# L-Scofano/SEEME

Measured on AMD Instinct MI355X. Metric: sampled seqs/sec (T=196, 50 DDIM steps), higher is better.
Workload: dtype f32 accumulate (fp16 denoiser weights, fp16 VAE MFMA operands); 1 GPU; config_mld_egobody interactee-only: VAE encode -> 50-step DDIM -> VAE decode, B=32/GPU, T=196, nfeats=132, random-init recipe weights; batch_per_gpu=32, seq_len=196, ddim_steps=50, parallelism=dp1 (independent shards, no collective on the data path)

## Files before the change

seeme_amd/csrc/den_cluster.inc.hip:

```cpp

#define DCL_MAGIC_EPOCH 0x7fffffffu
#define DCL_SPIN_LIMIT (1u << 22)

typedef __attribute__((address_space(1))) unsigned long long dcl_gu64;

template <typename WT> struct ClW {
    static constexpr int KL = WT::MFMA ? 32 : 16;
    static constexpr int UL = 256 / KL;
    static constexpr int RU = WT::MFMA ? 4 : 2;
    static constexpr unsigned UNIT_BYTES = 8u * UL * 1024u;
};
template <int C, bool Q = false> struct ClG {
    static constexpr int S = 256 / C;
    static constexpr int NB = 1024 / C;
    static constexpr int TA = S / 32;
    static constexpr int TB = 8 / C;
    static constexpr int U_A = 0, U_AS = TA, U_B = 2 * TA, U_C = U_B + TB;
    static constexpr int U_G = U_C + TB, U_H = U_G + 1;
    static constexpr int U_D = Q ? U_H + 2 : U_C + TB, U_E = U_D + 1, U_F = U_E + 1, NU_REAL = U_F + 2;
    static constexpr int NU = (NU_REAL + 3) / 4 * 4;
    static constexpr int SC = Q ? 8 : 4;
    static constexpr int X1_G = 2 * S + SC;
    static constexpr int G_BOOT = 0, G_X1 = 16, G_X2 = G_X1 + C * X1_G, G_X3 = G_X2 + C * 256, G_TOTAL = G_X3 + (Q ? C * 8 : 0);
    static constexpr int EPL = Q ? 3 : 2;
// ... 110 lines not shown
    }()), ...);
}
template <typename WT, int C, bool Q, int U0, int... Is>
__device__ __forceinline__ void cl_refills(ClRing<WT>& ring, int wave, unsigned voff, __amdgpu_buffer_rsrc_t rsrc, unsigned bc, unsigned bn,
                                           bool sc, bool sn, std::integer_sequence<int, Is...>) {
    (cl_issue<WT, C, Q, U0 + Is + ClW<WT>::RU>(ring, wave, voff, rsrc, bc, bn, sc, sn), ...);
    __builtin_amdgcn_sched_barrier(0);
}
constexpr int cl_clamp(int v, int lo, int hi) { return v < lo ? lo : (v > hi ? hi : v); }

#ifndef DCL_POLL_SLEEP
#define DCL_POLL_SLEEP 12
#endif
template <int... Us> using ClSeq = std::integer_sequence<int, Us...>;
template <int C, bool MF, bool Q> struct ClSched { static constexpr bool WIN = false; static constexpr int PRO = 0; typedef ClSeq<> W1A, W1B, W2A, W2B, WXA, WXB, W3, AF; };
template <> struct ClSched<8, true, false> { static constexpr bool WIN = true; static constexpr int PRO = 2; typedef ClSeq<> WXA, WXB; typedef ClSeq<2, 3> W1A; typedef ClSeq<4> W1B; typedef ClSeq<5> W2A; typedef ClSeq<6> W2B;
                                             typedef ClSeq<7> W3; typedef ClSeq<8, 9> AF; };
template <> struct ClSched<8, true, true> { static constexpr bool WIN = true; static constexpr int PRO = 2; typedef ClSeq<2, 3> W1A; typedef ClSeq<4> W1B; typedef ClSeq<5> W2A; typedef ClSeq<6> W2B;
                                            typedef ClSeq<7> WXA; typedef ClSeq<8> WXB; typedef ClSeq<9, 10> W3; typedef ClSeq<12, 13> AF; };
template <> struct ClSched<4, true, false> { static constexpr bool WIN = true; static constexpr int PRO = 4; typedef ClSeq<4, 5> W1A; typedef ClSeq<6, 7> W1B; typedef ClSeq<8, 9> W2A; typedef ClSeq<10, 11> W2B;
                                             typedef ClSeq<> WXA, WXB; typedef ClSeq<12, 13> W3; typedef ClSeq<14, 15> AF; };
template <> struct ClSched<4, true, true> { static constexpr bool WIN = true; static constexpr int PRO = 4; typedef ClSeq<4, 5> W1A; typedef ClSeq<6, 7> W1B; typedef ClSeq<8, 9> W2A; typedef ClSeq<10> W2B;
                                            typedef ClSeq<11> WXA; typedef ClSeq<12> WXB; typedef ClSeq<13, 14> W3; typedef ClSeq<16, 17, 18, 19> AF; };
template <typename WT, int C, bool Q, int... Us>
__device__ __forceinline__ void cl_issue_seq(ClRing<WT>& ring, int wave, unsigned voff, __amdgpu_buffer_rsrc_t rsrc, unsigned bc, unsigned bn,
                                             bool sc, bool sn, ClSeq<Us...>) {
    (cl_issue<WT, C, Q, Us>(ring, wave, voff, rsrc, bc, bn, sc, sn), ...);
    __builtin_amdgcn_sched_barrier(0);
}
typedef __attribute__((address_space(3))) volatile int cl_lds_flag;
__device__ __forceinline__ void cl_flag_set(int* f, unsigned v) { *(cl_lds_flag*)f = (int)v; }
__device__ __forceinline__ void cl_flag_wait(const int* f, unsigned v) {
    while (*(const cl_lds_flag*)f != (int)v) __builtin_amdgcn_s_sleep(1);
}

__device__ __forceinline__ void cl_store_granule(unsigned long long* g, unsigned epoch, float v, bool local) {
    const unsigned long long x = ((unsigned long long)epoch << 32) | __float_as_uint(v);
    if (local) *(volatile dcl_gu64*)g = x;
    else __hip_atomic_store((dcl_gu64*)g, x, __ATOMIC_RELAXED, __HIP_MEMORY_SCOPE_AGENT);
}
__device__ __forceinline__ unsigned cl_tags_ok(const u32x4& a, unsigned epoch) { return (unsigned)(a.y == epoch) & (unsigned)(a.w == epoch); }

template <int C> struct ClRes {
    static constexpr int S = ClG<C>::S, NB = ClG<C>::NB;
    static constexpr int SKIP_B = 0, IN_B = S;
    static constexpr int L1B = 4 * S;
    static constexpr int V5 = L1B + NB;
    static constexpr int F1B = V5 + 5 * 256;
    static constexpr int V4 = F1B + FF_D;
    static constexpr int CT = V4 + 4 * 256;
    static constexpr int LAYER = CT + 512;
    static constexpr int NL1 = NB > 256 ? NB / 256 : 1;
    static constexpr int NP = 16 + NL1;
    static constexpr int ROWS = 5 * 256;
    static constexpr int FLOATS = SEEME_DEN_NL * LAYER + 2 * ROWS;
};
template <int C>
__device__ __forceinline__ void cl_load_resident(int wave, int lane, float* __restrict__ res, const float* __restrict__ vpg, const DenLayout* __restrict__ lay,
                                                 const float* __restrict__ tt_row, const SeemeSampleArgs& A, int b, int c, int ca_R) {
    typedef ClRes<C> R;
    const uint32_t base = lds_addr_of(res);
#pragma unroll 1
    for (int p = wave; p < SEEME_DEN_NL * R::NP + 5; p += DEN_THREADS / 64) {
        const float* src; int d, n = 64;
        if (p >= SEEME_DEN_NL * R::NP) {
            const int j = p - SEEME_DEN_NL * R::NP;
// ... 48 lines not shown
        else if (i <= 15) { src = tt_row + l * 512 + (i - 14) * 256; d = VP_LAYER + (i - 14) * 256; n = 64; }
        else if (i <= 17) { src = tt_row + 2560 + l * 1024 + 512 + (i - 16) * 256; d = VP_LAYER + 1024 + (i - 16) * 256; n = 64; }
        else if (i < 18 + NL1) { d = (int)(L->l1b - L->skip_b) + c * G::NB + (i - 18) * 256; src = vb + d; n = G::NB >= 256 ? 64 : G::NB / 4; }
        else {
            const int j = i - 18 - NL1;
            if (j <= 1) { src = tt_row + 2560 + l * 1024 + j * 256; d = VP_LAYER + 512 + j * 256; n = 64; }
            else if (j <= 6) {
                const int64_t f = j == 2 ? L->cnw : j == 3 ? L->cnb : j == 4 ? L->csnw : j == 5 ? L->csnb : L->cao_b;
                d = (int)(f - L->skip_b); src = vb + d; n = 64;
            }
            else if (j == 7) { d = (int)(L->caq_b - L->skip_b) + c * G::S; src = vb + d; n = G::S / 4; }
            else if (j < 8 + 4 * A.N) {
                const int t = (j - 8) >> 2, q = (j - 8) & 3;
                src = A.ctab + ((size_t)b * A.N + t) * SEEME_CROW + (q < 2 ? l * 512 + q * 256 : 2560 + l * 512 + (q - 2) * 256);
                d = VP_LAYER + STG_TT + t * 1024 + q * 256; n = 64;
            }
        }
        dst = d; n4 = n;
        r = make_float4(0.f, 0.f, 0.f, 0.f);
        if (lane < n) r = *reinterpret_cast<const float4*>(src + 4 * lane);
    }
    __device__ __forceinline__ void store(int lane, float* __restrict__ stg) const {
        if (lane < n4) *reinterpret_cast<float4*>(stg + dst + 4 * lane) = r;
    }
};
#define DCL_MAX_N 2

template <typename WT, int C, bool Q>
__global__ __launch_bounds__(DEN_THREADS) void k_den_cluster(const ClArgs ka) {
    extern __shared__ __attribute__((aligned(16))) float smem[];
    typedef ClW<WT> W; typedef ClG<C, Q> G;
    constexpr int A_DEF0 = cl_clamp(2 * G::TA - W::RU, 0, 2 * G::TA);
    constexpr int A_INL0 = cl_clamp(A_DEF0, 0, G::TA), A_INL1 = cl_clamp(A_DEF0 - G::TA, 0, G::TA), C_INL = cl_clamp(G::TB - W::RU, 0, G::TB);
    typedef ClSched<C, WT::MFMA, Q> SCH;
    constexpr bool WIN = SCH::WIN;
    const SeemeSampleArgs& A = ka.s;
    const DenLayout* __restrict__ lay = &ka.lay;
    const float* __restrict__ vp = ka.vp;
    const int tid = threadIdx.x, lane = tid & 63;
    const int wave = __builtin_amdgcn_readfirstlane(tid >> 6);
    int b, c;
    if (ka.placement == 0) { const int x = blockIdx.x & 7, j = blockIdx.x >> 3; b = x * (ka.clusters / 8) + j / C; c = j % C; }
    else { b = blockIdx.x / C; c = blockIdx.x % C; }
    if (b >= A.B) return;
    const bool epi = wave == 0;
    const int N = Q ? A.N : 1;
    typedef ClRes<C> R;
    constexpr bool RSD = !Q;
    const int stg_sz = VP_LAYER + STG_TT + N * 1024;
    const int ca_R = A.trow_per_sample ? 1 : A.steps;

    float* CONSTV = smem;
    float* KEEP = CONSTV + 768;
    float* STG = KEEP + 256;
    float* ROWS = STG + SEEME_DEN_NL * R::LAYER;
    float* XA = STG + (RSD ? R::FLOATS : 2 * stg_sz);
    float* XB = XA + 512;
    float* XH = XB + 512;
    float* SKF = XH + 2 * (G::NB > 128 ? G::NB : 128);
    float* QS = SKF + 1024;
    float* KS = QS + G::S;
    float* PART = KS + G::S;
    float* RES = PART + 256;
    int* FLG = reinterpret_cast<int*>(RES + 256);
    constexpr int XZERO = 512 + 512 + 2 * (G::NB > 128 ? G::NB : 128) + 1024;

    const __amdgpu_buffer_rsrc_t wg = __builtin_amdgcn_make_buffer_rsrc(const_cast<void*>(ka.wgc), 0, (int)ka.wgc_bytes, 0x00020000);
    unsigned long long* const xg = ka.xg + (size_t)b * G::G_TOTAL;
    const __amdgpu_buffer_rsrc_t xr_ = __builtin_amdgcn_make_buffer_rsrc(xg, 0, G::G_TOTAL * 8, 0x00020000);
    const unsigned voff = (unsigned)wave * (unsigned)(W::UL * 1024) + (unsigned)lane * 16u;
    const int col = lane & 15;
    const ClX xa = cl_xin<WT>(XA, lane), xb = cl_xin<WT>(XB, lane), xh = cl_xin<WT>(XH, lane);
    const float sa_scale = 1.f / 16.f;
    if (epi) __builtin_amdgcn_s_setprio(3);

    typedef const __attribute__((address_space(4))) int32_t* CI32;
    typedef const __attribute__((address_space(4))) float* CF32;
    const CI32 trow_c = (CI32)(uintptr_t)A.trow;
    const CF32 coef_c = (CF32)(uintptr_t)A.coef;
    int row = A.trow_per_sample ? trow_c[b] : trow_c[0];

    float4 xr = ld4(A.latents + (size_t)b * 256 + 4 * lane);
    for (int i = tid; i < 192; i += DEN_THREADS)
        st4(CONSTV + 4 * i, i < 64 ? ld4(vp + lay->pe0 + 4 * i) : (i < 128 ? ld4(vp + lay->fnw + 4 * (i - 64)) : ld4(vp + lay->fnb + 4 * (i - 128))));
    if constexpr (RSD) cl_load_resident<C>(wave, lane, STG, vp, lay, A.ttab + (size_t)row * SEEME_TROW, A, b, c, ca_R);
    else stage_dma<1, Q, 0, 0>(wave, lane, STG, vp, &lay->L[0], A.ttab + (size_t)row * SEEME_TROW, 0, A, b, N, 0, ca_R);
    for (int i = tid; i < XZERO / 4; i += DEN_THREADS) st4(XA + 4 * i, make_float4(0.f, 0.f, 0.f, 0.f));
    if (tid >= 1 && tid < 4) FLG[tid] = 0;
    bool dead = false, local = false;
    if (epi) {
        const unsigned my_xcc = __builtin_amdgcn_s_getreg(0x1814) & 15u;
        if (lane == 0) cl_store_granule(xg + G::G_BOOT + c, DCL_MAGIC_EPOCH, __uint_as_float(my_xcc), false);
        unsigned spins = 0, idv = 0;
        for (;;) {
            const unsigned long long x = __hip_atomic_load((dcl_gu64*)(xg + G::G_BOOT + (lane % C)), __ATOMIC_RELAXED, __HIP_MEMORY_SCOPE_AGENT);
            idv = (unsigned)x;
            if (__all((unsigned)(x >> 32) == DCL_MAGIC_EPOCH)) break;
            if (++spins > DCL_SPIN_LIMIT) { dead = true; if (lane == 0) atomicOr(ka.hdr, 1u); break; }
            __builtin_amdgcn_s_sleep(2);
        }
        local = !dead && __all(idv == my_xcc) && !(ka.flags & 1);
        if (lane == 0) { FLG[0] = local ? 1 : 0; if (local && c == 0) atomicAdd(ka.hdr + 1, 1u); }
    }
    wait_vmcnt0();
    __syncthreads();
    local = FLG[0] != 0;
    if (epi) {
        st4(KEEP + 4 * lane, xr);
        xr = f4_add(xr, ld4(CONSTV + 4 * lane));
        put_x<WT, 1>(XA, 0, 0, lane, xr);
        st4(RES + 4 * lane, xr);
    }
    ClRing<WT> ring;
    {
        const unsigned b0 = (unsigned)((0 * C + c) * G::NU) * W::UNIT_BYTES;
        cl_issue<WT, C, Q, 0>(ring, wave, voff, wg, b0, b0, false, false);
        cl_issue<WT, C, Q, 1>(ring, wave, voff, wg, b0, b0, false, false);
        if constexpr (W::RU == 4 && (!WIN || SCH::PRO == 4)) { cl_issue<WT, C, Q, 2>(ring, wave, voff, wg, b0, b0, false, false); cl_issue<WT, C, Q, 3>(ring, wave, voff, wg, b0, b0, false, false); }
    }
    __syncthreads();
    int cur = 0;

#pragma unroll 1
    for (int step = 0; step < A.steps; ++step) {
        if (step == 2) DEN_DBG(1);
        if (step == 3) DEN_DBG(2);
        const int step_next = step + 1 < A.steps ? step + 1 : step;
        const int row_next = A.trow_per_sample ? row : trow_c[step_next];
#pragma unroll 1
        for (int l = 0; l < SEEME_DEN_NL; ++l) {
            const DenLayerOff* __restrict__ L = &lay->L[l];
            const int ln = (l + 1 < SEEME_DEN_NL) ? l + 1 : 0;
            const DenLayerOff* __restrict__ Ln = &lay->L[ln];
            const bool skip = l >= 3, nskip = ln >= 3;
            const unsigned bc = (unsigned)((l * C + c) * G::NU) * W::UNIT_BYTES, bn = (unsigned)((ln * C + c) * G::NU) * W::UNIT_BYTES;
            const float* VP = STG + (RSD ? l * R::LAYER : cur * stg_sz);
            const float* TTS = RSD ? ROWS + cur * R::ROWS : VP + VP_LAYER;
            const float* TFS = TTS + (RSD ? 512 : 1024);
            const float* CT = RSD ? VP + R::CT : TTS + STG_TT;
            const float* CA_ADD = TTS + 1024;
            constexpr int IN_ST = RSD ? G::S : 256;
            const int d0 = RSD ? 0 : c * G::S, j0 = RSD ? 0 : c * G::NB;
            const float* v_skip_b = RSD ? VP + R::SKIP_B : VP;
            const float* v_in_b = RSD ? VP + R::IN_B : VP + (L->in_b - L->skip_b);
            const float* v_n1w = RSD ? VP + R::V5 : VP + (L->n1w - L->skip_b), *v_n1b = RSD ? VP + R::V5 + 256 : VP + (L->n1b - L->skip_b);
            const float* v_l1b = RSD ? VP + R::L1B : VP + (L->l1b - L->skip_b), *v_l2b = RSD ? VP + R::V5 + 512 : VP + (L->l2b - L->skip_b);
            const float* v_n2w = RSD ? VP + R::V5 + 768 : VP + (L->n2w - L->skip_b), *v_n2b = RSD ? VP + R::V5 + 1024 : VP + (L->n2b - L->skip_b);
            const float* v_f1b = RSD ? VP + R::F1B : VP + (L->f1b - L->skip_b), *v_f2b = RSD ? VP + R::V4 : VP + (L->f2b - L->skip_b);
            const float* v_fsnw = RSD ? VP + R::V4 + 256 : VP + (L->fsnw - L->skip_b), *v_fsnb = RSD ? VP + R::V4 + 512 : VP + (L->fsnb - L->skip_b);
            const float* v_fo_b = RSD ? VP + R::V4 + 768 : VP + (L->fo_b - L->skip_b);
            const float* v_cnw = VP + (L->cnw - L->skip_b), *v_cnb = VP + (L->cnb - L->skip_b), *v_caq_b = VP + (L->caq_b - L->skip_b);
            const float* v_csnw = VP + (L->csnw - L->skip_b), *v_csnb = VP + (L->csnb - L->skip_b), *v_cao_b = VP + (L->cao_b - L->skip_b);
            (void)CA_ADD; (void)v_cnw; (void)v_cnb; (void)v_caq_b; (void)v_csnw; (void)v_csnb; (void)v_cao_b;
            const bool ywave = wave >= 6;
            const float* const tt_next = A.ttab + (size_t)(ln == 0 ? row_next : row) * SEEME_TROW;
            const int ca_next = A.trow_per_sample ? 0 : (ln == 0 ? step_next : step);
            ClStage<C, true> nxt;
            (void)nxt; (void)ca_next;
            const unsigned e1 = 1u + (unsigned)G::EPL * (unsigned)(step * SEEME_DEN_NL + l), e2 = e1 + 1u, e3 = e1 + 2u;
            (void)e3;

            {
                f32x4 acc[G::TA];
                cl_zero<G::TA>(acc);
                const bool act = skip || !ywave;
                cl_units<WT, C, Q, G::U_A, G::TA, G::TA, 0, 0, A_INL0>(ring, xa, acc, act, wave, voff, wg, bc, bn, skip, nskip, std::make_integer_sequence<int, G::TA>{});
                {
                    const ClX xs = cl_xin<WT>(SKF + (l == 3 ? 512 : 0), lane);
                    cl_units<WT, C, Q, G::U_AS, G::TA, G::TA, G::TA, W::UL, A_INL1>(ring, xs, acc, skip, wave, voff, wg, bc, bn, skip, nskip, std::make_integer_sequence<int, G::TA>{});
                }
                if (act && lane < 16) {
#pragma unroll
                    for (int t = 0; t < G::TA; ++t) {
                        const int T = wave * G::TA + t, part = T / (G::S / 16), d = (T % (G::S / 16)) * 16 + col, D = d0 + d;
                        const float val = cl_out<WT>(acc[t]);
                        const unsigned epoch = e1;
                        if (part == 0) QS[d] = val + v_in_b[D];
                        else if (part == 1) KS[d] = val + v_in_b[IN_ST + D];
                        else if (part == 2) cl_store_granule(xg + G::G_X1 + c * G::X1_G + d, epoch, val + v_in_b[2 * IN_ST + D], local);
                        else cl_store_granule(xg + G::G_X1 + c * G::X1_G + G::S + d, epoch, val + v_skip_b[D], local);
                    }
                }
            }
            __syncthreads(); DEN_DBG(0);
            if (epi) {
                const unsigned epoch = e1;
                constexpr int NT = Q ? DCL_MAX_N + 2 : 3;
                float ps[NT];
#pragma unroll
                for (int j = 0; j < NT; ++j) ps[j] = 0.f;
#pragma unroll
                for (int dd = 0; dd < G::S; dd += 64) {
                    const int d = dd + lane;
                    if (d < G::S) {
                        const float q = QS[d];
// ... 10 lines not shown
#pragma unroll
                    for (int j = 0; j < NT; ++j) pv = lane == j ? ps[j] : pv;
                    if (lane < G::SC) cl_store_granule(xg + G::G_X1 + c * G::X1_G + 2 * G::S + lane, epoch, pv, local);
                }
                if constexpr (WIN) {
                    __builtin_amdgcn_sched_barrier(0);
                    cl_issue_seq<WT, C, Q>(ring, wave, voff, wg, bc, bn, skip, nskip, typename SCH::W1A{});
                    if (lane == 0) cl_flag_set(FLG + 1, e1);
                    __builtin_amdgcn_s_sleep(DCL_POLL_SLEEP);
                }
                const int pub = (4 * lane) / G::S, off = (4 * lane) % G::S;
                const unsigned o_v = (unsigned)((G::G_X1 + pub * G::X1_G + off) * 8);
                const unsigned o_s = (unsigned)((G::G_X1 + (lane % C) * G::X1_G + 2 * G::S) * 8);
                u32x4 gv0, gv1, gy0, gy1, gs[G::SC / 2];
                gy0 = gy1 = u32x4{0u, epoch, 0u, epoch};
                unsigned spins = 0;
                for (;;) {
                    gv0 = __builtin_amdgcn_raw_buffer_load_b128(xr_, o_v, 0, 16);
                    gv1 = __builtin_amdgcn_raw_buffer_load_b128(xr_, o_v + 16, 0, 16);
                    if (skip) {
                        gy0 = __builtin_amdgcn_raw_buffer_load_b128(xr_, o_v + G::S * 8, 0, 16);
                        gy1 = __builtin_amdgcn_raw_buffer_load_b128(xr_, o_v + G::S * 8 + 16, 0, 16);
                    }
#pragma unroll
                    for (int j = 0; j < G::SC / 2; ++j) gs[j] = __builtin_amdgcn_raw_buffer_load_b128(xr_, o_s + 16 * j, 0, 16);
                    unsigned ok = cl_tags_ok(gv0, epoch) & cl_tags_ok(gv1, epoch) & cl_tags_ok(gy0, epoch) & cl_tags_ok(gy1, epoch);
#pragma unroll
                    for (int j = 0; j < G::SC / 2; ++j) ok &= cl_tags_ok(gs[j], epoch);
                    if (__all(ok != 0u) || dead) break;
                    if (++spins > DCL_SPIN_LIMIT) { dead = true; if (lane == 0) atomicOr(ka.hdr, 2u); break; }
                }
                if constexpr (WIN) {
                    cl_issue_seq<WT, C, Q>(ring, wave, voff, wg, bc, bn, skip, nskip, typename SCH::W1B{});
                    if (lane == 0) cl_flag_set(FLG + 2, e1);
                }
                DEN_DBG(0);
                float sc[NT];
#pragma unroll
                for (int j = 0; j < NT; ++j) {
                    sc[j] = __uint_as_float((j & 1) ? gs[j >> 1].z : gs[j >> 1].x);
                    if (C >= 2) sc[j] += dpp_f(sc[j], 0);
                    if (C >= 4) sc[j] += dpp_f(sc[j], 1);
                    if (C >= 8) sc[j] += dpp_f(sc[j], 2);
                }
                float mx = fmaxf(sc[0], sc[NT - 1]);
#pragma unroll
                for (int n = 0; n < NT - 2; ++n) if (n < N) mx = fmaxf(mx, sc[1 + n]);
                float esum = 0.f;
#pragma unroll
                for (int j = 0; j < NT; ++j) { sc[j] = (j == 0 || j == NT - 1 || j - 1 < N) ? fast_exp(sc[j] - mx) : 0.f; esum += sc[j]; }
                const float inv = fast_rcp(esum);
                const float4 vv = make_float4(__uint_as_float(gv0.x), __uint_as_float(gv0.z), __uint_as_float(gv1.x), __uint_as_float(gv1.z));
                float4 att = f4_scale(vv, sc[0] * inv);
#pragma unroll
                for (int n = 0; n < NT - 2; ++n) if (n < N) att = f4_fma(sc[1 + n] * inv, ld4(CT + n * 1024 + 256 + 4 * lane), att);
                att = f4_fma(sc[NT - 1] * inv, ld4(TTS + 256 + 4 * lane), att);
                if (skip) xr = make_float4(__uint_as_float(gy0.x), __uint_as_float(gy0.z), __uint_as_float(gy1.x), __uint_as_float(gy1.z));
                xr = wave_ln(f4_add(xr, att), v_n1w, v_n1b, lane);
                put_x<WT, 1>(XB, 0, 0, lane, xr);
            } else {
                ClRow nrow;
                if constexpr (WIN) cl_flag_wait(FLG + 1, e1);
                if constexpr (RSD) {
                    nrow.load(wave, lane, tt_next, A.catab + (((size_t)b * ca_R + ca_next) * SEEME_DEN_NL + ln) * 256, ln);
                    __builtin_amdgcn_sched_barrier(0);
                }
                if constexpr (WIN) {
                    cl_issue_seq<WT, C, Q>(ring, wave, voff, wg, bc, bn, skip, nskip, typename SCH::W1A{});
                    cl_flag_wait(FLG + 2, e1);
                    cl_issue_seq<WT, C, Q>(ring, wave, voff, wg, bc, bn, skip, nskip, typename SCH::W1B{});
                }
                if constexpr (RSD) nrow.store(wave, lane, ROWS + (cur ^ 1) * R::ROWS);
            }
            __syncthreads(); DEN_DBG(0);

            if constexpr (Q) nxt.load(0, wave, lane, vp, Ln, tt_next, ln, A, b, c, ca_next, ca_R);
            if constexpr (!WIN) cl_refills<WT, C, Q, G::U_A + A_DEF0>(ring, wave, voff, wg, bc, bn, skip, nskip, std::make_integer_sequence<int, 2 * G::TA - A_DEF0>{});
            {
                f32x4 acc[G::TB];
                cl_zero<G::TB>(acc);
                cl_units<WT, C, Q, G::U_B, G::TB, G::TB, 0, 0, (WIN ? 0 : G::TB)>(ring, xb, acc, true, wave, voff, wg, bc, bn, skip, nskip, std::make_integer_sequence<int, G::TB>{});
                if (lane < 16) {
#pragma unroll
                    for (int t = 0; t < G::TB; ++t) {
                        const int j = (wave * G::TB + t) * 16 + col;
                        cl_put1<WT>(XH, j, fmaxf(cl_out<WT>(acc[t]) + v_l1b[j0 + j], 0.f));
                    }
                }
            }
            if constexpr (Q) nxt.store(lane, STG + (cur ^ 1) * stg_sz);
            __syncthreads(); DEN_DBG(0);

            if constexpr (Q) nxt.load(1, wave, lane, vp, Ln, tt_next, ln, A, b, c, ca_next, ca_R);
            {
                f32x4 acc[2];
                cl_zero<2>(acc);
                cl_units<WT, C, Q, G::U_C, G::TB, 2, 0, 0, C_INL>(ring, xh, acc, true, wave, voff, wg, bc, bn, skip, nskip, std::make_integer_sequence<int, G::TB>{});
                if (lane < 32) {
                    const float val = (lane & 16) ? cl_out<WT>(acc[1]) : cl_out<WT>(acc[0]);
                    cl_store_granule(xg + G::G_X2 + c * 256 + (2 * wave + (lane >> 4)) * 16 + col, e2, val, local);
                }
            }
            if constexpr (Q) nxt.store(lane, STG + (cur ^ 1) * stg_sz);
            if (epi) {
                const unsigned epoch = e2;
                if constexpr (WIN) {
                    __builtin_amdgcn_sched_barrier(0);
                    cl_issue_seq<WT, C, Q>(ring, wave, voff, wg, bc, bn, skip, nskip, typename SCH::W2A{});
                    if (lane == 0) cl_flag_set(FLG + 1, e2);
                    __builtin_amdgcn_s_sleep(DCL_POLL_SLEEP);
                }
                float4 sum;
                unsigned spins = 0;
                for (;;) {
                    u32x4 g[C][2];
#pragma unroll
                    for (int p = 0; p < C; ++p) {
                        const unsigned o = (unsigned)((G::G_X2 + p * 256 + 4 * lane) * 8);
                        g[p][0] = __builtin_amdgcn_raw_buffer_load_b128(xr_, o, 0, 16);
                        g[p][1] = __builtin_amdgcn_raw_buffer_load_b128(xr_, o + 16, 0, 16);
                    }
                    unsigned ok = 1u;
                    sum = make_float4(0.f, 0.f, 0.f, 0.f);
#pragma unroll
                    for (int p = 0; p < C; ++p) {
                        ok &= cl_tags_ok(g[p][0], epoch) & cl_tags_ok(g[p][1], epoch);
                        sum.x += __uint_as_float(g[p][0].x); sum.y += __uint_as_float(g[p][0].z);
// ... 110 lines not shown
                            if (C >= 4) t += dpp_f(t, 1);
                            if (C >= 8) t += dpp_f(t, 2);
                            y = f4_fma(t * rL, ld4(CT + n * 1024 + 768 + 4 * lane), y);
                        }
                    }
                    const float4 hh = f4_adaln(wave_ln(y, v_csnw, v_csnb, lane), ld4(TTS + 512 + 4 * lane), ld4(TTS + 768 + 4 * lane));
                    put_x<WT, 1>(XB, 0, 0, lane, f4_silu(hh));
                } else if constexpr (WIN) {
                    cl_flag_wait(FLG + 1, e3);
                    cl_issue_seq<WT, C, Q>(ring, wave, voff, wg, bc, bn, skip, nskip, typename SCH::WXA{});
                    cl_flag_wait(FLG + 2, e3);
                    cl_issue_seq<WT, C, Q>(ring, wave, voff, wg, bc, bn, skip, nskip, typename SCH::WXB{});
                }
                __syncthreads(); DEN_DBG(0);
                if constexpr (!WIN) cl_refills<WT, C, Q, G::U_G>(ring, wave, voff, wg, bc, bn, skip, nskip, std::make_integer_sequence<int, 1>{});
                nxt.load(2, wave, lane, vp, Ln, tt_next, ln, A, b, c, ca_next, ca_R);
                {
                    f32x4 acc[2];
                    cl_zero<2>(acc);
                    cl_units<WT, C, Q, G::U_H, 2, 2, 0, 0, (WIN ? 0 : 2)>(ring, xb, acc, true, wave, voff, wg, bc, bn, skip, nskip, std::make_integer_sequence<int, 2>{});
                    if (lane < 32) {
                        const int n = (2 * wave + (lane >> 4)) * 16 + col;
                        const float x3 = RES[n] + ((lane & 16) ? cl_out<WT>(acc[1]) : cl_out<WT>(acc[0])) + v_cao_b[n];
                        RES[n] = x3;
                        cl_put1<WT>(XA, n, x3);
                    }
                }
                nxt.store(lane, STG + (cur ^ 1) * stg_sz);
                __syncthreads(); DEN_DBG(0);
            }

            if constexpr (Q) nxt.load(3, wave, lane, vp, Ln, tt_next, ln, A, b, c, ca_next, ca_R);
            if constexpr (!Q && !WIN) cl_refills<WT, C, Q, G::U_C + C_INL>(ring, wave, voff, wg, bc, bn, skip, nskip, std::make_integer_sequence<int, G::TB - C_INL>{});
            {
                f32x4 acc[1];
                cl_zero<1>(acc);
                cl_units<WT, C, Q, G::U_D, 1, 1, 0, 0, (WIN ? 0 : 1)>(ring, xa, acc, true, wave, voff, wg, bc, bn, skip, nskip, std::make_integer_sequence<int, 1>{});
                if (lane < 16) {
                    const int j = wave * 16 + col;
                    cl_put1<WT>(XH, j, fast_gelu(cl_out<WT>(acc[0]) + v_f1b[j]));
                }
            }
            if constexpr (Q) nxt.store(lane, STG + (cur ^ 1) * stg_sz);
            __syncthreads(); DEN_DBG(0);
            {
                f32x4 acc[2];
                cl_zero<2>(acc);
                cl_units<WT, C, Q, G::U_E, 1, 2, 0, 0, (WIN ? 0 : 1)>(ring, xh, acc, true, wave, voff, wg, bc, bn, skip, nskip, std::make_integer_sequence<int, 1>{});
                if (lane < 32) PART[(2 * wave + (lane >> 4)) * 16 + col] = (lane & 16) ? cl_out<WT>(acc[1]) : cl_out<WT>(acc[0]);
            }
            __syncthreads(); DEN_DBG(0);
            if (epi) {
                if constexpr (WIN) {
                    cl_issue_seq<WT, C, Q>(ring, wave, voff, wg, bc, bn, skip, nskip, typename SCH::W3{});
                    if (lane == 0) cl_flag_set(FLG + 3, e2);
                }
                const float4 y2 = f4_add(ld4(PART + 4 * lane), ld4(v_f2b + 4 * lane));
                const float4 hh = f4_adaln(wave_ln(y2, v_fsnw, v_fsnb, lane), ld4(TFS + 4 * lane), ld4(TFS + 256 + 4 * lane));
                put_x<WT, 1>(XB, 0, 0, lane, f4_silu(hh));
            } else if constexpr (WIN) {
                cl_flag_wait(FLG + 3, e2);
                cl_issue_seq<WT, C, Q>(ring, wave, voff, wg, bc, bn, skip, nskip, typename SCH::W3{});
            }
            __syncthreads(); DEN_DBG(0);
            if constexpr (Q) nxt.load(4, wave, lane, vp, Ln, tt_next, ln, A, b, c, ca_next, ca_R);
            if constexpr (WIN) __builtin_amdgcn_sched_barrier(0);
            {
                f32x4 acc[2];
                cl_zero<2>(acc);
                cl_units<WT, C, Q, G::U_F, 2, 2, 0, 0, (WIN ? 0 : 2)>(ring, xb, acc, true, wave, voff, wg, bc, bn, skip, nskip, std::make_integer_sequence<int, 2>{});
                if constexpr (WIN) cl_issue_seq<WT, C, Q>(ring, wave, voff, wg, bc, bn, skip, nskip, typename SCH::AF{});
                if (lane < 32) {
                    const int n = (2 * wave + (lane >> 4)) * 16 + col;
                    const float xn = RES[n] + ((lane & 16) ? cl_out<WT>(acc[1]) : cl_out<WT>(acc[0])) + v_fo_b[n];
                    RES[n] = xn;
                    cl_put1<WT>(XA, n, xn);
                    if (l < 2) cl_put1<WT>(SKF + 512 * l, n, xn);
                }
            }
            if constexpr (Q) nxt.store(lane, STG + (cur ^ 1) * stg_sz);
            if constexpr (!WIN) cl_refills<WT, C, Q, G::NU_REAL>(ring, wave, voff, wg, bc, bn, skip, nskip, std::make_integer_sequence<int, G::NU - G::NU_REAL>{});
            __syncthreads(); DEN_DBG(0);
            if (l + 1 < SEEME_DEN_NL) {
                if (epi && !nskip) xr = ld4(RES + 4 * lane);
            } else {
                if (epi) {
                    float4 e = wave_ln(ld4(RES + 4 * lane), CONSTV + 256, CONSTV + 512, lane);
                    if (A.sched == SEEME_SCHED_NONE) {
                        st4(KEEP + 4 * lane, e);
                    } else {
                        const CF32 cf = coef_c + (size_t)step * 8;
                        const float c0 = cf[0], c1 = cf[1], c2 = cf[2], c3 = cf[3], c4 = cf[4], c5 = cf[5], clip = cf[6], ptype = cf[7];
                        float4 nz = make_float4(0.f, 0.f, 0.f, 0.f);
                        if (A.noise != nullptr) nz = ld4(A.noise + ((size_t)step * A.B + b) * 256 + 4 * lane);
                        const float4 lat = ld4(KEEP + 4 * lane);
                        const float xs[4] = {lat.x, lat.y, lat.z, lat.w}, es4[4] = {e.x, e.y, e.z, e.w}, ns[4] = {nz.x, nz.y, nz.z, nz.w};
                        float o[4];
#pragma unroll
                        for (int i = 0; i < 4; ++i) {
                            float x0, ep;
                            if (ptype == 0.f) { ep = es4[i]; x0 = (xs[i] - c1 * ep) / c0; }
                            else              { x0 = es4[i]; ep = (xs[i] - c0 * x0) / c1; }
                            if (clip != 0.f) x0 = fminf(fmaxf(x0, -1.f), 1.f);
                            o[i] = c2 * x0 + c3 * ep + c5 * xs[i] + c4 * ns[i];
                        }
                        const float4 nl = make_float4(o[0], o[1], o[2], o[3]);
                        st4(KEEP + 4 * lane, nl);
                        xr = f4_add(nl, ld4(CONSTV + 4 * lane));
                        put_x<WT, 1>(XA, 0, 0, lane, xr);
                        st4(RES + 4 * lane, xr);
                    }
                }
                __syncthreads(); DEN_DBG(0);
            }
            cur ^= 1;
        }
        row = row_next;
    }
    DEN_DBG(3);
    if (epi && c == 0) st4(A.out + (size_t)b * 256 + 4 * lane, ld4(KEEP + 4 * lane));
#pragma unroll
    for (int s = 0; s < W::RU; ++s) asm volatile("" ::"v"(ring.r[s][0].x));
}

template <int C>
static size_t cl_lds_bytes(int N, bool q) {
    typedef ClG<C> G;
    const int stg = q ? 2 * (VP_LAYER + STG_TT + N * 1024) : ClRes<C>::FLOATS;
    return (size_t)(768 + 256 + stg + 512 + 512 + 2 * (G::NB > 128 ? G::NB : 128) + 1024 + 2 * G::S + 256 + 256 + 4) * sizeof(float);
}

extern "C" size_t seeme_den_cluster_xchg_bytes(int B, int C) {
    const size_t per = C == 8 ? ClG<8, true>::G_TOTAL : (C == 4 ? ClG<4, true>::G_TOTAL : ClG<2, true>::G_TOTAL);
    const size_t clusters = (size_t)(B + 7) / 8 * 8;
    return DCL_HDR_BYTES + clusters * per * 8;
}
extern "C" int seeme_den_cluster_layout(int C, int wdtype, int query, int64_t* out, int cap) {
    if (cap < 14) return seeme_fail("den_cluster_layout: output too small");
    if (C != 2 && C != 4 && C != 8) return seeme_fail("den_cluster_layout: C must be 2, 4 or 8");
    const int TA = 256 / C / 32, TB = 8 / C;
    const int u_c = 2 * TA + TB, u_g = u_c + TB, u_d = query ? u_g + 3 : u_g;
    const int64_t NU = (u_d + 4 + 3) / 4 * 4, UL = wdtype == 0 ? 16 : 8, UB = 8 * UL * 1024;
    out[0] = NU; out[1] = UB; out[2] = (int64_t)SEEME_DEN_NL * C * NU * UB; out[3] = UL; out[4] = 256 / UL;
    out[5] = 0; out[6] = TA; out[7] = 2 * TA; out[8] = u_c; out[9] = u_d; out[10] = u_d + 1; out[11] = u_d + 2;
    out[12] = query ? u_g : -1; out[13] = query ? u_g + 1 : -1;
    return 0;
}

template <typename WT, int C, bool Q>
static int launch_den_cluster(const ClArgs& ka0, hipStream_t st) {
    ClArgs ka = ka0;
    ka.clusters = (ka.s.B + 7) / 8 * 8;
    const int grid = ka.clusters * C;
    int dev = 0, cus = 0;
    SEEME_HIP(hipGetDevice(&dev));
// ... 51 lines not shown
```

seeme_amd/mld_denoiser.py:

```python
from __future__ import annotations

import ctypes as C
import math
import os
from typing import Optional

import torch
import torch.nn as nn

from . import _lib as L
from .mld_vae import _PositionEmbeddingLearned1D, _EncoderLayerParams, _SkipStackParams, _param_fingerprint

_LAYER_FIELDS = ["skip", "inp", "outp", "l1", "l2", "caq", "cao", "f1", "f2", "fo",
                 "skip_b", "in_b", "out_b", "n1w", "n1b", "l1b", "l2b", "n2w", "n2b", "cnw", "cnb", "caq_b",
                 "csnw", "csnb", "cao_b", "f1b", "f2b", "fsnw", "fsnb", "fo_b"]


_CUS = {}


def _device_cus(device) -> int:
    idx = torch.device(device).index
    idx = torch.cuda.current_device() if idx is None else idx
    if idx not in _CUS:
# ... 297 lines not shown
                    if query:
                        Wq_ca = blk.ca_block.query.weight.detach()[c * S:(c + 1) * S]
                        Wq_pad = torch.zeros(128, 256, dtype=Wq_ca.dtype, device=dev)
                        Wq_pad[:S] = Wq_ca
                        img[l, c, U_G:U_G + 1] = pack_stage(Wq_pad.to(wdt), 1)
                        img[l, c, U_H:U_H + 2] = pack_stage(blk.ca_block.proj_out.out_layers[2].weight.detach().to(wdt), 2)
                    u0 = U_D
                    img[l, c, u0:u0 + 1] = pack_stage(Wf1.to(wdt), 1)
                    img[l, c, u0 + 1:u0 + 2] = pack_stage(Wf2.to(wdt), 2)
                    img[l, c, u0 + 2:u0 + 4] = pack_stage(Wfo.to(wdt), 2)
        assert img.numel() * img.element_size() == total
        self._ccache[(Cc, query)] = (img, vpc, code)
        return self._ccache[(Cc, query)]

    def _cluster_size(self, B: int, N: int, cfg: bool, cus: int = 256) -> int:
        want = os.environ.get("SEEME_DEN_CLUSTER")
        want = self.cluster if want is None else (want if want == "auto" else int(want))
        if want == 0 or N > 2 or cfg or self.num_heads != 1:
            return 0
        Bp = (B + 7) // 8 * 8
        cus = min(int(cus), 256)
        if want == "auto":
            for Cc in (8, 4, 2):
                if Bp * Cc <= cus:
                    return Cc
            return 0
        return want if Bp * want <= cus else 0

    def _cluster_plan(self, B: int, N: int, cfg: bool, per_sample: bool, cus: int = 256):
        Cc = self._cluster_size(B, N, cfg, cus)
        want = os.environ.get("SEEME_DEN_CLUSTER")
        want = self.cluster if want is None else (want if want == "auto" else int(want))
        ms = os.environ.get("SEEME_DEN_CLUSTER_MS", "1") != "0" and self.cluster_ms
        if (want != "auto" or not ms or B <= 32 or N not in (1, 2) or cfg or per_sample or self.num_heads != 1
                or self.weight_dtype not in ("fp16", "bf16")):
            return Cc, 1
        forced = os.environ.get("SEEME_DEN_CLUSTER_MS_PLAN")
        if forced:
            C4, spc = (int(x) for x in forced.split(","))
            return C4, spc
        cus = min(int(cus), 256)
        if B <= 64 and Cc == 4:
            return Cc, 1
        ncl = (cus // 4) // 8 * 8
        most = 4 if self.weight_dtype == "bf16" else (8 if N == 1 else 6)
        if ncl >= 8 and -(-B // ncl) <= most:
            return 4, max(2, -(-B // ncl))
        return Cc, 1

    def cluster_status(self):
        if self._xchg is None:
            return (0, 0)
        hdr = self._xchg[:8].cpu().view(torch.int32)
        return int(hdr[0]), int(hdr[1])

    def _workspace(self, rows: int, device):
        need = L.lib().seeme_denoiser_workspace_bytes(rows, 0, 0)
        if self._ws is None or self._ws.numel() < need or self._ws.device != device:
            self._ws = torch.empty(need, dtype=torch.uint8, device=device)
        return self._ws

    def time_tables(self, tfeat: torch.Tensor) -> torch.Tensor:
        L.require_cuda(tfeat, "tfeat")
        tfeat = tfeat.contiguous()
        rows = tfeat.shape[0]
        ttab = torch.empty(rows, L.TROW, device=tfeat.device, dtype=torch.float32)
        ws = self._workspace(rows, tfeat.device)
        w = self._weights()
        L.check(L.lib().seeme_denoiser_time_tables(C.byref(w), tfeat.data_ptr(), rows, ttab.data_ptr(),
                                                    ws.data_ptr(), ws.numel(), L.current_stream()),
# ... 108 lines not shown
```

Measured before the change: 15350 seqs/s.

## Split C=8 cluster waves into two groups with separate weight-prefetch ring

For the C=8, 16-bit MFMA, non-query denoiser cluster kernel, the waves split into two groups of four. Waves 0-3 run the attention and input-projection stages, and waves 4-7 run the FFN and MLP stages. Each group streams its weights through its own two-slot register ring with explicit issue points, replacing the previous per-wave staggered schedule. The goal is to overlap weight streaming with compute across the two groups and to cut per-wave register ring depth, at the cost of extra syncthreads and flag waits. Separately, the Python planner now lets a forced multi-sample plan apply even when B<=32.

```diff
diff --git a/seeme_amd/csrc/den_cluster.inc.hip b/seeme_amd/csrc/den_cluster.inc.hip
--- a/seeme_amd/csrc/den_cluster.inc.hip
+++ b/seeme_amd/csrc/den_cluster.inc.hip
@@ -166,6 +166,50 @@
 __device__ __forceinline__ void cl_flag_set(int* f, unsigned v) { *(cl_lds_flag*)f = (int)v; }
 __device__ __forceinline__ void cl_flag_wait(const int* f, unsigned v) {
     while (*(const cl_lds_flag*)f != (int)v) __builtin_amdgcn_s_sleep(1);
+}
+
+template <typename WT, int C, bool Q> struct ClGrp { static constexpr bool ON = C == 8 && WT::MFMA && !Q; };
+struct ClSchedGrp { static constexpr bool WIN = true; static constexpr int PRO = 0; typedef ClSeq<> W1A, W1B, W2A, W2B, WXA, WXB, W3, AF; };
+struct ClRing2 { u32x4 r[2][2][8]; };
+#define DCLG_NOWHERE 0x7fff0000u
+template <int SLOT, int H = 3>
+__device__ __forceinline__ void clg_issue(ClRing2& ring, unsigned voff, __amdgpu_buffer_rsrc_t rsrc, unsigned soff, bool on0, bool on1) {
+    if constexpr (H & 1) {
+        const unsigned v0 = on0 ? voff : DCLG_NOWHERE;
+#pragma unroll
+        for (int i = 0; i < 8; ++i) ring.r[SLOT][0][i] = __builtin_amdgcn_raw_buffer_load_b128(rsrc, v0, soff + (unsigned)(i * 1024), 0);
+    }
+    if constexpr (H & 2) {
+        const unsigned v1 = on1 ? voff + 4u * 8u * 1024u : DCLG_NOWHERE;
+#pragma unroll
+        for (int i = 0; i < 8; ++i) ring.r[SLOT][1][i] = __builtin_amdgcn_raw_buffer_load_b128(rsrc, v1, soff + (unsigned)(i * 1024), 0);
+    }
+    __builtin_amdgcn_sched_barrier(0);
+}
+template <typename WT, int TPW, int J0, int KBOFF>
+__device__ __forceinline__ void clg_consume(const u32x4 (&slot)[2][8], const ClX& x, f32x4 (&acc)[2][TPW]) {
+    static_assert(WT::MFMA, "16-bit images only");
+    uint4 a4 = make_uint4(0u, 0u, 0u, 0u);
+#pragma unroll
+    for (int i = 0; i < 8; ++i) {
+        const int j = J0 + i, kb = j / TPW - KBOFF, t = j % TPW;
+        if (i == 0 || t == 0) a4 = *reinterpret_cast<const uint4*>(x.base + x.foff + kb * x.kbs);
+#pragma unroll
+        for (int h = 0; h < 2; ++h) {
+            if constexpr (WT::HALF) acc[h][t] = __builtin_amdgcn_mfma_f32_16x16x32_f16(__builtin_bit_cast(h16x8, a4), __builtin_bit_cast(h16x8, slot[h][i]), acc[h][t], 0, 0, 0);
+            else acc[h][t] = __builtin_amdgcn_mfma_f32_16x16x32_bf16(__builtin_bit_cast(bf16x8, a4), __builtin_bit_cast(bf16x8, slot[h][i]), acc[h][t], 0, 0, 0);
+        }
+    }
+}
+template <typename WT, int TPW>
+__device__ __forceinline__ float clg_out(const f32x4 (&acc)[2][TPW], int lane) {
+    const int h = TPW == 2 ? lane >> 5 : lane >> 4, t = TPW == 2 ? (lane >> 4) & 1 : 0;
+    float v = cl_out<WT>(acc[0][0]);
+#pragma unroll
+    for (int hh = 0; hh < 2; ++hh)
+#pragma unroll
+        for (int tt = 0; tt < TPW; ++tt) v = (h == hh && t == tt) ? cl_out<WT>(acc[hh][tt]) : v;
+    return v;
 }
 
 __device__ __forceinline__ void cl_store_granule(unsigned long long* g, unsigned epoch, float v, bool local) {
@@ -280,7 +324,8 @@
     typedef ClW<WT> W; typedef ClG<C, Q> G;
     constexpr int A_DEF0 = cl_clamp(2 * G::TA - W::RU, 0, 2 * G::TA);
     constexpr int A_INL0 = cl_clamp(A_DEF0, 0, G::TA), A_INL1 = cl_clamp(A_DEF0 - G::TA, 0, G::TA), C_INL = cl_clamp(G::TB - W::RU, 0, G::TB);
-    typedef ClSched<C, WT::MFMA, Q> SCH;
+    constexpr bool GRP = ClGrp<WT, C, Q>::ON;
+    typedef std::conditional_t<GRP, ClSchedGrp, ClSched<C, WT::MFMA, Q>> SCH;
     constexpr bool WIN = SCH::WIN;
     const SeemeSampleArgs& A = ka.s;
     const DenLayout* __restrict__ lay = &ka.lay;
@@ -317,6 +362,8 @@
     unsigned long long* const xg = ka.xg + (size_t)b * G::G_TOTAL;
     const __amdgpu_buffer_rsrc_t xr_ = __builtin_amdgcn_make_buffer_rsrc(xg, 0, G::G_TOTAL * 8, 0x00020000);
     const unsigned voff = (unsigned)wave * (unsigned)(W::UL * 1024) + (unsigned)lane * 16u;
+    const int w4 = wave & 3;
+    const unsigned gvoff = (unsigned)w4 * (unsigned)(W::UL * 1024) + (unsigned)lane * 16u;
     const int col = lane & 15;
     const ClX xa = cl_xin<WT>(XA, lane), xb = cl_xin<WT>(XB, lane), xh = cl_xin<WT>(XH, lane);
     const float sa_scale = 1.f / 16.f;
@@ -360,7 +407,14 @@
         st4(RES + 4 * lane, xr);
     }
     ClRing<WT> ring;
-    {
+    ClRing2 gr;
+    (void)gr; (void)gvoff; (void)w4;
+    if constexpr (GRP) {
+        if (wave < 4) {
+            clg_issue<0>(gr, gvoff, wg, (unsigned)(c * G::NU + G::U_A) * W::UNIT_BYTES, true, w4 < 2);
+            clg_issue<1>(gr, gvoff, wg, (unsigned)(c * G::NU + G::U_AS) * W::UNIT_BYTES, false, false);
+        }
+    } else {
         const unsigned b0 = (unsigned)((0 * C + c) * G::NU) * W::UNIT_BYTES;
         cl_issue<WT, C, Q, 0>(ring, wave, voff, wg, b0, b0, false, false);
         cl_issue<WT, C, Q, 1>(ring, wave, voff, wg, b0, b0, false, false);
@@ -408,7 +462,88 @@
             const unsigned e1 = 1u + (unsigned)G::EPL * (unsigned)(step * SEEME_DEN_NL + l), e2 = e1 + 1u, e3 = e1 + 2u;
             (void)e3;
 
-            {
+            if constexpr (GRP) {
+                if (wave >= 4) {
+                    __syncthreads();
+                    {
+                        ClRow nrow;
+                        cl_flag_wait(FLG + 1, e1);
+                        nrow.load(wave, lane, tt_next, A.catab + (((size_t)b * ca_R + ca_next) * SEEME_DEN_NL + ln) * 256, ln);
+                        __builtin_amdgcn_sched_barrier(0);
+                        clg_issue<0>(gr, gvoff, wg, bc + (unsigned)G::U_B * W::UNIT_BYTES, true, true);
+                        nrow.store(wave, lane, ROWS + (cur ^ 1) * R::ROWS);
+                    }
+                    __syncthreads();
+                    {
+                        f32x4 acc[2][1];
+                        cl_zero<1>(acc[0]); cl_zero<1>(acc[1]);
+                        clg_consume<WT, 1, 0, 0>(gr.r[0], xb, acc);
+                        cl_pin<1>(acc[0]); cl_pin<1>(acc[1]);
+                        if (lane < 32) {
+                            const int j = (w4 + 4 * (lane >> 4)) * 16 + col;
+                            cl_put1<WT>(XH, j, fmaxf(clg_out<WT, 1>(acc, lane) + v_l1b[j], 0.f));
+                        }
+                    }
+                    __syncthreads();
+                    cl_flag_wait(FLG + 1, e2);
+                    clg_issue<1>(gr, gvoff, wg, bc + (unsigned)G::U_D * W::UNIT_BYTES, true, true);
+                    cl_flag_wait(FLG + 2, e2);
+                    clg_issue<0>(gr, gvoff, wg, bc + (unsigned)G::U_F * W::UNIT_BYTES, true, true);
+                    __syncthreads();
+                    {
+                        f32x4 acc[2][1];
+                        cl_zero<1>(acc[0]); cl_zero<1>(acc[1]);
+                        clg_consume<WT, 1, 0, 0>(gr.r[1], xa, acc);
+                        cl_pin<1>(acc[0]); cl_pin<1>(acc[1]);
+                        if (lane < 32) {
+                            const int j = (w4 + 4 * (lane >> 4)) * 16 + col;
+                            cl_put1<WT>(XH, j, fast_gelu(clg_out<WT, 1>(acc, lane) + v_f1b[j]));
+                        }
+                    }
+                    __syncthreads();
+                    clg_issue<1, 1>(gr, gvoff, wg, bc + (unsigned)(G::U_F + 1) * W::UNIT_BYTES, true, true);
+                    __syncthreads();
+                    clg_issue<1, 2>(gr, gvoff, wg, bc + (unsigned)(G::U_F + 1) * W::UNIT_BYTES, true, true);
+                    __syncthreads();
+                    {
+                        f32x4 acc[2][2];
+                        cl_zero<2>(acc[0]); cl_zero<2>(acc[1]);
+                        clg_consume<WT, 2, 0, 0>(gr.r[0], xb, acc);
+                        cl_pin<2>(acc[0]); cl_pin<2>(acc[1]);
+                        clg_consume<WT, 2, W::UL, 0>(gr.r[1], xb, acc);
+                        cl_pin<2>(acc[0]); cl_pin<2>(acc[1]);
+                        const int n = (2 * (w4 + 4 * (lane >> 5)) + ((lane >> 4) & 1)) * 16 + col;
+                        const float xn = RES[n] + clg_out<WT, 2>(acc, lane) + v_fo_b[n];
+                        RES[n] = xn;
+                        cl_put1<WT>(XA, n, xn);
+                        if (l < 2) cl_put1<WT>(SKF + 512 * l, n, xn);
+                    }
+                    __syncthreads();
+                    if (l + 1 == SEEME_DEN_NL) __syncthreads();
+                    cur ^= 1;
+                    continue;
+                }
+            }
+
+            if constexpr (GRP) {
+                f32x4 acc[2][1];
+                cl_zero<1>(acc[0]); cl_zero<1>(acc[1]);
+                clg_consume<WT, 1, 0, 0>(gr.r[0], xa, acc);
+                cl_pin<1>(acc[0]); cl_pin<1>(acc[1]);
+                if (skip) {
+                    const ClX xs = cl_xin<WT>(SKF + (l == 3 ? 512 : 0), lane);
+                    clg_consume<WT, 1, W::UL, W::UL>(gr.r[1], xs, acc);
+                }
+                cl_pin<1>(acc[0]); cl_pin<1>(acc[1]);
+                if (lane < 32) {
+                    const int sw = w4 + 4 * (lane >> 4), d = (sw & 1) * 16 + col;
+                    const float val = clg_out<WT, 1>(acc, lane);
+                    if (sw < 2) QS[d] = val + v_in_b[d];
+                    else if (sw < 4) KS[d] = val + v_in_b[IN_ST + d];
+                    else if (sw < 6) cl_store_granule(xg + G::G_X1 + c * G::X1_G + d, e1, val + v_in_b[2 * IN_ST + d], local);
+                    else if (skip) cl_store_granule(xg + G::G_X1 + c * G::X1_G + G::S + d, e1, val + v_skip_b[d], local);
+                }
+            } else {
                 f32x4 acc[G::TA];
                 cl_zero<G::TA>(acc);
                 const bool act = skip || !ywave;
@@ -485,6 +620,7 @@
                 }
                 if constexpr (WIN) {
                     cl_issue_seq<WT, C, Q>(ring, wave, voff, wg, bc, bn, skip, nskip, typename SCH::W1B{});
+                    if constexpr (GRP) clg_issue<0>(gr, gvoff, wg, bc + (unsigned)G::U_C * W::UNIT_BYTES, true, true);
                     if (lane == 0) cl_flag_set(FLG + 2, e1);
                 }
                 DEN_DBG(0);
@@ -522,6 +658,7 @@
                     cl_issue_seq<WT, C, Q>(ring, wave, voff, wg, bc, bn, skip, nskip, typename SCH::W1A{});
                     cl_flag_wait(FLG + 2, e1);
                     cl_issue_seq<WT, C, Q>(ring, wave, voff, wg, bc, bn, skip, nskip, typename SCH::W1B{});
+                    if constexpr (GRP) clg_issue<0>(gr, gvoff, wg, bc + (unsigned)G::U_C * W::UNIT_BYTES, true, true);
                 }
                 if constexpr (RSD) nrow.store(wave, lane, ROWS + (cur ^ 1) * R::ROWS);
             }
@@ -529,7 +666,9 @@
 
             if constexpr (Q) nxt.load(0, wave, lane, vp, Ln, tt_next, ln, A, b, c, ca_next, ca_R);
             if constexpr (!WIN) cl_refills<WT, C, Q, G::U_A + A_DEF0>(ring, wave, voff, wg, bc, bn, skip, nskip, std::make_integer_sequence<int, 2 * G::TA - A_DEF0>{});
-            {
+            if constexpr (GRP) {
+                clg_issue<1>(gr, gvoff, wg, bc + (unsigned)G::U_E * W::UNIT_BYTES, true, true);
+            } else {
                 f32x4 acc[G::TB];
                 cl_zero<G::TB>(acc);
                 cl_units<WT, C, Q, G::U_B, G::TB, G::TB, 0, 0, (WIN ? 0 : G::TB)>(ring, xb, acc, true, wave, voff, wg, bc, bn, skip, nskip, std::make_integer_sequence<int, G::TB>{});
@@ -545,7 +684,13 @@
             __syncthreads(); DEN_DBG(0);
 
             if constexpr (Q) nxt.load(1, wave, lane, vp, Ln, tt_next, ln, A, b, c, ca_next, ca_R);
-            {
+            if constexpr (GRP) {
+                f32x4 acc[2][2];
+                cl_zero<2>(acc[0]); cl_zero<2>(acc[1]);
+                clg_consume<WT, 2, 0, 0>(gr.r[0], xh, acc);
+                cl_pin<2>(acc[0]); cl_pin<2>(acc[1]);
+                cl_store_granule(xg + G::G_X2 + c * 256 + (2 * (w4 + 4 * (lane >> 5)) + ((lane >> 4) & 1)) * 16 + col, e2, clg_out<WT, 2>(acc, lane), local);
+            } else {
                 f32x4 acc[2];
                 cl_zero<2>(acc);
                 cl_units<WT, C, Q, G::U_C, G::TB, 2, 0, 0, C_INL>(ring, xh, acc, true, wave, voff, wg, bc, bn, skip, nskip, std::make_integer_sequence<int, G::TB>{});
@@ -722,7 +867,9 @@
 
             if constexpr (Q) nxt.load(3, wave, lane, vp, Ln, tt_next, ln, A, b, c, ca_next, ca_R);
             if constexpr (!Q && !WIN) cl_refills<WT, C, Q, G::U_C + C_INL>(ring, wave, voff, wg, bc, bn, skip, nskip, std::make_integer_sequence<int, G::TB - C_INL>{});
-            {
+            if constexpr (GRP) {
+                clg_issue<0>(gr, gvoff, wg, bn + (unsigned)G::U_A * W::UNIT_BYTES, true, nskip || w4 < 2);
+            } else {
                 f32x4 acc[1];
                 cl_zero<1>(acc);
                 cl_units<WT, C, Q, G::U_D, 1, 1, 0, 0, (WIN ? 0 : 1)>(ring, xa, acc, true, wave, voff, wg, bc, bn, skip, nskip, std::make_integer_sequence<int, 1>{});
@@ -733,7 +880,13 @@
             }
             if constexpr (Q) nxt.store(lane, STG + (cur ^ 1) * stg_sz);
             __syncthreads(); DEN_DBG(0);
-            {
+            if constexpr (GRP) {
+                f32x4 acc[2][2];
+                cl_zero<2>(acc[0]); cl_zero<2>(acc[1]);
+                clg_consume<WT, 2, 0, 0>(gr.r[1], xh, acc);
+                cl_pin<2>(acc[0]); cl_pin<2>(acc[1]);
+                PART[(2 * (w4 + 4 * (lane >> 5)) + ((lane >> 4) & 1)) * 16 + col] = clg_out<WT, 2>(acc, lane);
+            } else {
                 f32x4 acc[2];
                 cl_zero<2>(acc);
                 cl_units<WT, C, Q, G::U_E, 1, 2, 0, 0, (WIN ? 0 : 1)>(ring, xh, acc, true, wave, voff, wg, bc, bn, skip, nskip, std::make_integer_sequence<int, 1>{});
@@ -755,7 +908,9 @@
             __syncthreads(); DEN_DBG(0);
             if constexpr (Q) nxt.load(4, wave, lane, vp, Ln, tt_next, ln, A, b, c, ca_next, ca_R);
             if constexpr (WIN) __builtin_amdgcn_sched_barrier(0);
-            {
+            if constexpr (GRP) {
+                clg_issue<1>(gr, gvoff, wg, bn + (unsigned)G::U_AS * W::UNIT_BYTES, nskip, nskip);
+            } else {
                 f32x4 acc[2];
                 cl_zero<2>(acc);
                 cl_units<WT, C, Q, G::U_F, 2, 2, 0, 0, (WIN ? 0 : 2)>(ring, xb, acc, true, wave, voff, wg, bc, bn, skip, nskip, std::make_integer_sequence<int, 2>{});
@@ -809,8 +964,13 @@
     }
     DEN_DBG(3);
     if (epi && c == 0) st4(A.out + (size_t)b * 256 + 4 * lane, ld4(KEEP + 4 * lane));
-#pragma unroll
-    for (int s = 0; s < W::RU; ++s) asm volatile("" ::"v"(ring.r[s][0].x));
+    if constexpr (GRP) {
+#pragma unroll
+        for (int s = 0; s < 2; ++s) asm volatile("" ::"v"(gr.r[s][0][0].x));
+    } else {
+#pragma unroll
+        for (int s = 0; s < W::RU; ++s) asm volatile("" ::"v"(ring.r[s][0].x));
+    }
 }
 
 template <int C>
diff --git a/seeme_amd/mld_denoiser.py b/seeme_amd/mld_denoiser.py
--- a/seeme_amd/mld_denoiser.py
+++ b/seeme_amd/mld_denoiser.py
@@ -353,10 +353,10 @@
         want = os.environ.get("SEEME_DEN_CLUSTER")
         want = self.cluster if want is None else (want if want == "auto" else int(want))
         ms = os.environ.get("SEEME_DEN_CLUSTER_MS", "1") != "0" and self.cluster_ms
-        if (want != "auto" or not ms or B <= 32 or N not in (1, 2) or cfg or per_sample or self.num_heads != 1
+        forced = os.environ.get("SEEME_DEN_CLUSTER_MS_PLAN")
+        if (want != "auto" or not ms or (B <= 32 and not forced) or N not in (1, 2) or cfg or per_sample or self.num_heads != 1
                 or self.weight_dtype not in ("fp16", "bf16")):
             return Cc, 1
-        forced = os.environ.get("SEEME_DEN_CLUSTER_MS_PLAN")
         if forced:
             C4, spc = (int(x) for x in forced.split(","))
             return C4, spc
```

Measured after the change: 16410 seqs/s (median of 6 runs). 1.07x the previous value.
